# szbonaldo/FedMLP

Measured on AMD Instinct MI355X. Metric: images/sec/client (ICH 224x224 bs=128) at 1/2/4/8 GPUs; mAP vs ref, higher is better.
Workload: dtype f32; 1 GPU; FedMLP stage1 step, Resnet18, ICH-shaped synthetic 3x224x224, C=5, bs=128, one client per GPU, FedAvg all-reduce every 40 steps + once at end; parallelism=clients1, rccl_ranks=1, stream_mode=default: frozen teacher + weight gradients on the engine's side stream, arithmetic=fp32 operands+sums; products as 6 exact bf16 partials on the bf16 matrix pipe

## Files before the change

fedmlp_amd/_lib.py:

```python
import ctypes as C
import os

_HERE = os.path.dirname(os.path.abspath(__file__))
LIB_PATH = os.environ.get("FEDMLP_HIP_LIB") or os.path.join(_HERE, "libfedmlp_hip.so")

FM_MAX_CLASSES = 32
FM_MAX_GROUPS = 8
FM_COMM_ID_BYTES = 128


class FmConfig(C.Structure):
    _fields_ = [("model", C.c_int32), ("n_classes", C.c_int32), ("in_h", C.c_int32),
                ("in_w", C.c_int32), ("max_images", C.c_int32), ("reserved", C.c_int32 * 3),
                ("stream", C.c_void_p)]


class FmAdam(C.Structure):
    _fields_ = [("lr", C.c_float), ("beta1", C.c_float), ("beta2", C.c_float),
                ("eps", C.c_float), ("weight_decay", C.c_float)]


class FmSgd(C.Structure):
    _fields_ = [("lr", C.c_float), ("momentum", C.c_float), ("dampening", C.c_float),
                ("weight_decay", C.c_float), ("nesterov", C.c_int32)]
# ... 98 lines not shown
    "fm_debug_conv_fwd": (C.c_int, [_P, _I32, _P, _P, _I32, _I32, _P, _P, _P, _I32, _P, _P, _P, _P]),
    "fm_debug_block_dgrad": (C.c_int, [_P, _I32, _P, _P, _P, _I32]),
    "fm_debug_conv_planes": (C.c_int, [_P, _I32, _P, _I32, _P, _P, _P, _P, _I32, _P, _P]),
    "fm_debug_conv_arm": (C.c_int, [_P, _I32, _I32, _I32]),
    "fm_debug_pw": (C.c_int, [_P, _I32, _I32, _P, _P, _P, _I32, _I32, _P, _P, _P, _P]),
    "fm_debug_pw_fwd": (C.c_int, [_P, _I32, _P, _P, _I32, _I32, _P, _P, _P, _I32, _P, _P, _P, _P]),
    "fm_debug_proj_bwd": (C.c_int, [_P, _I32, _I32, _P, _P, _P, _P, _P, _I32, _I32, _P, _P]),
    "fm_debug_exp_bwd": (C.c_int, [_P, _I32, _P, _P, _P, _P, _P, _I32, _I32, _P, _P]),
    "fm_debug_get_grads": (C.c_int, [_P, _P]),
    "fm_debug_optim_arena": (C.c_int, [_P, _I32, C.POINTER(_P), C.POINTER(_I64)]),
    "fm_debug_entry_spans": (C.c_int, [_P, _P, _I32]),
    "fm_debug_activation": (C.c_int, [_P, _I32, _I32, _I32, _P, C.POINTER(_I32)]),
    "fm_debug_stem_masks": (C.c_int, [_P, _I32, _I32, _P, _P]),
    "fm_debug_lose_part": (C.c_int, [_I32]),
    "fm_debug_ew": (C.c_int, [_P, _I32, C.POINTER(_P), C.POINTER(_I32), _F]),
    "fm_debug_eff": (C.c_int, [_P, _I32, C.POINTER(_P), C.POINTER(_I32), _F]),
    "fm_debug_eff_ws": (C.c_int, [_I32, C.POINTER(_I32), C.POINTER(C.c_int64)]),
    "fm_debug_head": (C.c_int, [_P, _I32, C.POINTER(_P), C.POINTER(_I32), _F]),
}

_lib = None


def load():
    global _lib
    if _lib is not None:
        return _lib
    if not os.path.exists(LIB_PATH):
        raise RuntimeError(
            f"{LIB_PATH} is missing: the HIP extension is not built and fedmlp_amd has no CPU "
# ... 32 lines not shown
```

fedmlp_amd/csrc/engine.hip:

```cpp
#include <math.h>
#include <stdio.h>
#include <string.h>

#include <algorithm>
#include <string>
#include <unordered_map>
#include <vector>

#include "../../include/fedmlp_hip.h"
#include "../../include/fedmlp_hip_debug.h"
#include "comm.h"
#include "common.h"
#include "kernels.h"
#include "pwconv.h"

static thread_local std::string g_err;
const char* fm_last_error(void) { return g_err.c_str(); }
const char* fm_version(void) { return "fedmlp_hip 0.2 (gfx950)"; }

#define HIPCHK(x)                                                                              \
    do {                                                                                       \
        hipError_t e_ = (x);                                                                   \
        if (e_ != hipSuccess) {                                                                \
            char b_[512];                                                                      \
// ... 157 lines not shown
    size_t NP = 0, NS = 0;
    size_t off_fcw = 0, off_fcb = 0, off_gamma = 0, off_beta = 0, off_rm = 0, off_rv = 0;
    int64_t nf_sd = 0, ni_sd = 0;
    float *grad = nullptr, *adam_m = nullptr, *adam_v = nullptr;
    float* stage_sd = nullptr;
    fm_adam hp{3e-5f, 0.9f, 0.999f, 1e-8f, 5e-4f};
    int64_t adam_t = 0;
    float *x4 = nullptr, *dyh0 = nullptr;
    float* x3 = nullptr;
    bool stem_rows = false;
    unsigned short* x3p = nullptr;
    long long x3p_plane_elems = 0;
    uint8_t* idx0 = nullptr;
    float *GA = nullptr, *GB = nullptr, *GC = nullptr, *GD = nullptr, *GE = nullptr;
    float *ws_stats = nullptr, *ws_part = nullptr;
    int stats_conv = -1, stats_tiles_n = 0;
    size_t slab_floats = 0;
    float *ca = nullptr, *cb = nullptr, *cc = nullptr;
    float *feat = nullptr, *logits = nullptr, *tfeat = nullptr, *tlogits = nullptr, *dlogits = nullptr;
    float* psum = nullptr;
    int64_t *pcnt = nullptr, *tcnt = nullptr;
    float* zeros = nullptr;
    int *sel_counts = nullptr, *sel_top = nullptr, *sel_bot = nullptr, *cls_dev = nullptr;
    int sel_cap = 0;
    int* tag_buf = nullptr;
    size_t tag_buf_ints = 0;
    bool prof = false, prof_fail = false;
    hipError_t soft_err = hipSuccess;
    int* dev_err = nullptr;
    int* host_err = nullptr;
    int* host_err_dev = nullptr;
    bool oprof = false;
    int ctx = -1;
// ... 656 lines not shown
        DALLOC(e->GA, pooled); DALLOC(e->GB, pooled); DALLOC(e->GC, pooled); DALLOC(e->GD, pooled); DALLOC(e->GE, pooled);
    } else {
        const EffSizes z = eff_sizes(e);
        AALLOC(e->GA, z.g_io); AALLOC(e->GB, z.g_io);
        AALLOC(e->T_small, z.t_small); AALLOC(e->T_big, z.t_big);
        DALLOC(e->se_dgp, B * z.max_ce); DALLOC(e->se_drp, B * z.max_cs); DALLOC(e->se_ds, B * z.max_ce);
        side = side && side_fits(e);
        DALLOC(e->hfeat, B * e->D);
    }
    DALLOC(e->ws_stats, max_stats);
    DALLOC(e->ws_part, (size_t)2 * (1024 + 32) * 2 * e->maxC);
    e->slab_floats = std::max<size_t>(max_slab * 8, (size_t)48 << 20);
    DALLOC(e->main.ws_slab, e->slab_floats);
    e->main.rec = e->main.ws_slab;
    DALLOC(e->ca, 2 * e->maxC); DALLOC(e->cb, 2 * e->maxC); DALLOC(e->cc, 2 * e->maxC);
    DALLOC(e->feat, B * e->D); DALLOC(e->tfeat, B * e->D);
    DALLOC(e->logits, B * e->C); DALLOC(e->tlogits, B * e->C); DALLOC(e->dlogits, B * e->C);
    DALLOC(e->psum, (size_t)2 * e->C * e->D); DALLOC(e->pcnt, 2 * e->C); DALLOC(e->tcnt, e->C);
    DALLOC(e->sel_counts, 2); DALLOC(e->cls_dev, FM_MAX_CLASSES);
    DALLOC(e->zeros, 64);
    if (e->planes) {
        const size_t pooled = B * (c0.hout / 2) * (c0.wout / 2) * 64;
        PALLOC(e->GBp, pooled); PALLOC(e->GCp, pooled); PALLOC(e->GDp, pooled);
        size_t mx = 0;
        for (auto& c : e->convs) {
            if (c.cin == 3) continue;
            mx = std::max(mx, std::max(B * c.hin * c.win * c.cin_p, B * c.hout * c.wout * c.cout_p));
        }
        e->xp_scratch_elems = mx * 3;
        float* t3 = nullptr;
// ... 440 lines not shown
            int imgs_per_group, bool frozen, bool z_is_relu_of_bn = false, unsigned short* dyp = nullptr, const unsigned short* zh = nullptr)
{
    const Conv& c = e->convs[bi];
    Bn& b = e->bns[bi];
    const int pix = imgs_per_group * c.hout * c.wout;
    const char* fy = getenv("FM_BN_MASK_FROM_Y");
    const int from_y = fy ? atoi(fy) : 1;
    const float *msc = nullptr, *msh = nullptr;
    if (z_is_relu_of_bn && (z || zh) && (from_y || !z)) { msc = b.scale; msh = b.shift; z = nullptr; zh = nullptr; }
    k_bn_bwd_reduce(dz, z, c.y, b.mean, b.istd, e->ws_part, groups, pix, b.C, L.st, msc, msh, zh);
    k_bn_bwd_finalize(e->ws_part, groups, bn_bwd_blocks(pix), b.C, pix, e->student.state + e->off_gamma + b.ch_off, b.mean,
                      b.istd, e->ca, e->cb, e->cc, e->grad + e->off_gamma + b.ch_off,
                      e->grad + e->off_beta + b.ch_off, L.st, frozen);
    if (dyp) k_bn_bwd_apply_planes(dz, z, c.y, e->ca, e->cb, e->cc, dy, dyp, dyh_out, groups, pix, b.C, L.st, msc, msh, zh);
    else k_bn_bwd_apply(dz, z, c.y, e->ca, e->cb, e->cc, dy, dyh_out, groups, pix, b.C, L.st, msc, msh);
}

void to_nhwc4(fm_engine* e, Lane& L, const float* const* xs, int groups, int B)
{
    if (e->precision && e->model == 1) {
        const Conv& c = e->convs[e->c_stem];
        for (int g = 0; g < groups; ++g)
            k_stem_im2col(xs[g], reinterpret_cast<bf16*>(e->stem_col) + (size_t)g * B * c.hout * c.wout * c.Kw, B, e->H, e->W, c.hout,
                          c.wout, c.k, c.stride, c.pad, c.pad, L.st);
        return;
    }
    if (e->convs[0].stem3) {
        const Conv& c = e->convs[0];
        for (int g = 0; g < groups; ++g)
            k_frame_nhwc3(xs[g], e->x3 + (size_t)g * B * c.Hp * c.Wp * 3, B, e->H, e->W, c.Hp, c.Wp, 3, 3, 0, L.st,
// ... 386 lines not shown
    if (first > nb + 1) return;
    e->ctx = 500;
    { OP(L, "k_fc_bwd"); k_fc_bwd(e->dlogits, e->feat, S + e->off_fcw, nullptr, e->grad + e->off_fcw, e->grad + e->off_fcb, e->GA, DT_F32, imgs,
             512, e->C, cl.hout * cl.wout, L.st, bw.dfeat); }
    float *ga = e->GA, *ge = e->GE;
    for (int b = nb - 1; b >= 0 && 1 + b >= first; --b) {
        const Block& blk = e->blocks[b];
        e->ctx = 400 + b;
        const BlockActs& a = A.blk[b];
        const int par = b & 1;
        float *GB = GBp[par], *GC = GCp[par], *GD = GDp[par];
        unsigned short *gbp = pm ? PB[par] : nullptr, *gcp = pm ? PC[par] : nullptr, *gdp = pm ? PD[par] : nullptr;
        const float* in = b == 0 ? A.p0 : A.blk[b - 1].out;
        const bool last = b + 1 == (int)e->blocks.size();
        side_guard(e, 0, par);
        { OP(L, "bn_bwd");
          if (pm && !last) bn_bwd(e, L, blk.c2, ga, nullptr, nullptr, ga, groups, B, bw.frozen, false, gbp, a.outp);
          else bn_bwd(e, L, blk.c2, ga, a.out, pm ? nullptr : GB, ga, groups, B, bw.frozen, false, gbp); }
        if (blk.ds >= 0) { side_guard(e, 1, par); OP(L, "bn_bwd"); bn_bwd(e, L, blk.ds, ga, nullptr, pm ? nullptr : GC, nullptr, groups, B, bw.frozen, false, gcp); }
        side_guard(e, 2, par);
        { OP(L, "conv_dgrad"); conv_dgrad(e, L, blk.c2, GB, GD, imgs, nullptr, false, gbp); }
        if (conv_on(e, tr, blk.c2)) {
            Lane& SL = side(0, par);
            { OP(SL, "conv_wgrad"); conv_wgrad(e, SL, blk.c2, a.z1, GB, imgs, nullptr, 0, pm ? a.z1p : nullptr, gbp); }
            side_end(e, 0, par);
        }
        { OP(L, "bn_bwd");
          if (pm) bn_bwd(e, L, blk.c1, GD, nullptr, nullptr, nullptr, groups, B, bw.frozen, true, gdp, a.z1p);
          else bn_bwd(e, L, blk.c1, GD, a.z1, GD, nullptr, groups, B, bw.frozen, true); }
        { OP(L, "conv_dgrad");
          if (blk.ds >= 0) {
              if (!block_dgrad(e, L, blk.c1, blk.ds, GD, GC, ge, imgs, gdp, gcp)) {
                  conv_dgrad(e, L, blk.ds, GC, ge, imgs, nullptr, false, gcp);
                  conv_dgrad(e, L, blk.c1, GD, ge, imgs, nullptr, true, gdp);
// ... 2195 lines not shown
        k_bn_bwd_finalize(F(0), d[0], d[1], d[2], d[3], F(1), F(2), F(3), F(4), F(5), F(6), F(7), F(8), s, d[4] != 0);
        break;
    case FM_EW_BN_BWD_APPLY:
    case FM_EW_BN_BWD_APPLY_PLANES: {
        const bool pl = op == FM_EW_BN_BWD_APPLY_PLANES;
        ARGCHK(need({0, 2, 3, 4, 5}) && pos(3) && d[2] % 4 == 0 && (!p[8] == !p[9]), "bn_bwd_apply: C % 4, mask_scale with mask_shift");
        if (pl) {
            ARGCHK(d[2] % 32 == 0 && p[10], "bn_bwd_apply_planes: C % 32, dyp");
            k_bn_bwd_apply_planes(F(0), F(1), F(2), F(3), F(4), F(5), F(6), U(10), F(7), d[0], d[1], d[2], s, F(8), F(9), U(11));
        } else {
            ARGCHK(p[6], "bn_bwd_apply: dy");
            k_bn_bwd_apply(F(0), F(1), F(2), F(3), F(4), F(5), F(6), F(7), d[0], d[1], d[2], s, F(8), F(9));
        }
        break;
    }
    default:
        ARGCHK(false, "op");
    }
    HIPCHK(hipGetLastError());
    HIPCHK(hipStreamSynchronize(s));
    return FM_OK;
}

static const char* eff_dims_bad(int32_t op, const int32_t* d)
{
    auto pos = [&](int a, int b) { for (int i = a; i < b; ++i) if (d[i] < 1) return false; return true; };
    if (op == FM_EFF_DW_FWD || op == FM_EFF_DW_DGRAD || op == FM_EFF_DW_WGRAD) {
        if (d[0] != DT_F32 && d[0] != DT_BF16) return "dt";
        if (!pos(1, 7) || d[12] < 1) return "a dimension < 1";
        if (d[6] % 4) return "C % 4";
        if (d[7] != 3 && d[7] != 5) return "K is 3 or 5";
        if (d[8] != 1 && d[8] != 2) return "stride is 1 or 2";
        if (d[4] != (d[2] + d[8] - 1) / d[8] || d[5] != (d[3] + d[8] - 1) / d[8]) return "Ho, Wo = ceil(Hi, Wi / stride)";
        if (d[9] < 0 || d[9] >= d[7] || d[10] < 0 || d[10] >= d[7]) return "pad_t, pad_l in 0 .. K-1";
        if (d[11] < 0 || d[11] > 2) return "act";
// ... 214 lines not shown
```

fedmlp_amd/csrc/kernels.h:

```cpp
#pragma once
#include <hip/hip_runtime.h>
#include <stdint.h>

#include "common.h"

#define FM_MAXC 32

struct ClassVec { float v[FM_MAXC]; };
struct TapList { int t[9]; int n; };

void k_nchw_to_nhwc4(const float* x, float* y, int imgs, int H, int W, hipStream_t s);
void k_stem_im2col(const float* x, void* col, int imgs, int H, int W, int Ho, int Wo, int k, int stride, int pad_t, int pad_l,
                   hipStream_t s);
void k_oihw_to_ohwi(const float* src, float* dst, int O, int I, int H, int W, int Wpad, int Ipad, hipStream_t s, int Ostride = 0);
void k_ohwi_to_oihw(const float* src, float* dst, int O, int I, int H, int W, int Wpad, int Ipad, hipStream_t s, int Ostride = 0);
void k_stem3_mask_grad(float* g, int O, hipStream_t s);
void k_frame_nhwc3(const float* x, float* y, int imgs, int H, int W, int Hp, int Wp, int top, int left, int src_nhwc3,
                   hipStream_t s, unsigned short* yp = nullptr, long long yp_plane_elems = 0);
void k_pack_dgrad(const float* w, float* out, int Co, int T, int Ci, TapList taps, hipStream_t s);
struct PackJob { long long w_off; float* out; int Co, T, Ci, ntaps; int taps[9]; int blk0; };
void k_pack_dgrad_all(const float* state, const PackJob* jobs, int njobs, int nblocks, hipStream_t s);
int pack_job_blocks(int Co, int Ci, int ntaps);
struct SplitJob { long long src_off; const float* src; long long dst_off; int M, nkb, blk0; };
void k_split_weights(const float* src_base, unsigned short* dst_base, const SplitJob* jobs, int njobs, int nblocks, hipStream_t s);
int split_job_blocks(int M, int nkb);
struct SplitJobBM { long long src_off; const float* src; long long dst_off; int M, ntaps, cib, blk0; };
void k_split_weights_bm(const float* src_base, unsigned short* dst_base, const SplitJobBM* jobs, int njobs, int nblocks, hipStream_t s);
int split_job_bm_blocks(int M, int nsteps);
void k_split_planes(const float* x, unsigned short* dst, long long npix, int C, hipStream_t s);
void k_planes_to_f32(const unsigned short* src, float* x, long long npix, int C, hipStream_t s);
void k_bn_apply_planes(const float* y, const float* scale, const float* shift, const float* res, const float* y2, const float* scale2,
                       const float* shift2, float* out, unsigned short* outp, int groups, int pix_per_group, int C, int relu,
                       hipStream_t s, const unsigned short* resp = nullptr);
void k_stem_pool_planes(const float* y, const float* scale, const float* shift, float* pooled, uint8_t* idx, unsigned short* pooledp,
                        int groups, int imgs_per_group, int H, int W, int C, hipStream_t s);
void k_bn_bwd_apply_planes(const float* dz, const float* z, const float* y, const float* ca, const float* cb, const float* cc, float* dy,
                           unsigned short* dyp, float* dyh_out, int groups, int pix_per_group, int C, hipStream_t s,
                           const float* mask_scale = nullptr, const float* mask_shift = nullptr, const unsigned short* zh = nullptr);
void k_scale(float* x, float w, int64_t n, hipStream_t s);
#define FM_FOLD_MAX 16
struct FoldArgs { const float* s[FM_FOLD_MAX]; float n[FM_FOLD_MAX]; };
void k_fedavg_fold(const FoldArgs& a, int K, float tot, float* out, int64_t n, hipStream_t s);
void k_axpby(float* y, const float* x, float a, float b, int64_t n, hipStream_t s);
#define FM_DIST_CHUNK 8192
struct DistEntry { long long off; int len, row, dense, Ipad, I, Wpad, W, chunk0, nchunks, all_real; };
struct DistChunk { int entry, start; };
void k_state_dist(const FoldArgs& a, int K, const float* ref, const DistEntry* ent, int n_entries, const DistChunk* chunks,
                  int n_chunks, int64_t NS, double* part, float* norms, hipStream_t s);

#define FM_METRICS_ROWS 64
#define FM_METRICS_BP 256
#define FM_METRICS_TILE 2048
size_t fm_metrics_ws_bytes(int64_t N, int C);
// ... 171 lines not shown
```

fedmlp_amd/csrc/planes_ew.hip:

```cpp
#include "common.h"
#include "kernels.h"
#include "split3.h"

static inline int pe_cdiv(int64_t a, int64_t b) { return (int)((a + b - 1) / b); }

#if __HIP_DEVICE_COMPILE__
__device__ __forceinline__ size_t pe_off(int c, int64_t pix, int64_t P)
{
    return (((size_t)(c >> 5) * 3) * P + pix) * 64 + ((c & 15) >> 2) * 16 + ((c >> 4) & 1) * 8;
}
__device__ __forceinline__ void pe_store_planes(unsigned short* planes, int64_t P, int c, int64_t pix, f32x4 v, bool active)
{
    f32x4 up;
#pragma unroll
    for (int k = 0; k < 4; ++k) up[k] = __shfl_down(v[k], 4);
    if (active && (c & 16) == 0) {
        sp_u32x4 H, M, L;
        split3(v, up, H, M, L);
        unsigned char* d = reinterpret_cast<unsigned char*>(planes) + (((size_t)(c >> 5) * 3) * P + pix) * 64 + ((c & 15) >> 2) * 16;
        *reinterpret_cast<sp_u32x4*>(d) = H;
        *reinterpret_cast<sp_u32x4*>(d + (size_t)P * 64) = M;
        *reinterpret_cast<sp_u32x4*>(d + (size_t)P * 128) = L;
    }
}
// ... 163 lines not shown
    if (active) {
        if (dyh_out) st4(dyh_out + o, d);
        if (dy) st4(dy + o, r);
    }
    pe_store_planes(dyp, P, c, pix, r, active);
#endif
}
void k_bn_bwd_apply_planes(const float* dz, const float* z, const float* y, const float* ca, const float* cb, const float* cc, float* dy,
                           unsigned short* dyp, float* dyh_out, int groups, int pix_per_group, int C, hipStream_t s,
                           const float* mask_scale, const float* mask_shift, const unsigned short* zh)
{
    const int64_t n4 = (int64_t)pix_per_group * (C / 4);
    hipLaunchKernelGGL(bn_bwd_apply_planes_kernel, dim3(pe_cdiv(n4, 256), groups), dim3(256), 0, s, dz, z, y, ca, cb, cc, dy, dyp,
                       dyh_out, pix_per_group, C, mask_scale, mask_shift, zh);
}
```

fedmlp_amd/csrc/pwgrad.hip:

```cpp
#include <stdlib.h>

#include <algorithm>
#include <type_traits>

#include "common.h"
#include "kernels.h"
#include "split3.h"

#if __HIP_DEVICE_COMPILE__
template <int IMM> __device__ __forceinline__ uint2 pw_read_tr(unsigned addr)
{
    uint2 v;
    asm volatile("ds_read_b64_tr_b16 %0, %1 offset:%2" : "=v"(v) : "v"(addr), "n"(IMM));
    return v;
}
#endif

template <int N, typename F> __device__ __forceinline__ void pw_for(F f)
{
    f(std::integral_constant<int, 0>{});
    if constexpr (N > 1) f(std::integral_constant<int, 1>{});
    if constexpr (N > 2) f(std::integral_constant<int, 2>{});
    if constexpr (N > 3) f(std::integral_constant<int, 3>{});
}
template <int FR, int FC, int SP>
__global__ __launch_bounds__(512, 2) void pwgrad_kernel(const PwgradParams p)
{
#if __HIP_DEVICE_COMPILE__
    constexpr int WN = 4;
    constexpr int BM = 32 * FR, BN = 64 * FC;
    constexpr int NBA = BM / 32, NBB = BN / 32;
    constexpr int SA = NBA * 6144, SB = NBB * 6144;
    constexpr int JA = (NBA * 3 + 3) / 4, JB = (NBB * 3 + 3) / 4;
    typedef __attribute__((address_space(3))) void lds_void;
    extern __shared__ __attribute__((aligned(16))) unsigned char smem[];
    const int tid = threadIdx.x;
    const int lane = tid & 63, wave = __builtin_amdgcn_readfirstlane(tid >> 6);
    const int wm = wave / WN, wn = wave % WN;
    const int li = lane & 15, lg = lane >> 4;
    const unsigned lds0 = (unsigned)(size_t)smem;
    const unsigned As = lds0, Bs = lds0 + 2 * SA;

    const int tile = blockIdx.x, split = blockIdx.y;
    const int tm = tile % p.tilesM, tn = tile / p.tilesM;
    const int m0 = tm * BM;
    const int jb0 = tn * NBB;
    const int cib = p.Ci >> 5;
    const long long pbeg = (long long)split * p.pix_per_split;
    const long long pend = min(p.npix, pbeg + p.pix_per_split);
    const int nsteps = (int)((pend - pbeg + 31) >> 5);
    const int Wi = p.Wi, Hi = p.Hi, Wo = p.Wo, Ho = p.Ho;

    constexpr unsigned OOB = 0x80000000u;
    const int h16 = wave & 1, q4 = wave >> 1;
    const int drow = 16 * h16 + (lane >> 2);
    const int chunk = (lane & 3) ^ (((drow >> 3) & 1) << 1);
    const __amdgpu_buffer_rsrc_t rsA = __builtin_amdgcn_make_buffer_rsrc(
        const_cast<unsigned short*>(p.dYp), 0, (unsigned)((size_t)(p.M >> 5) * 3 * p.npix * 64), 0x00020000);
    const int shift = p.pad * (Wi + 1);
    const __amdgpu_buffer_rsrc_t rsB = __builtin_amdgcn_make_buffer_rsrc(
        const_cast<unsigned char*>(reinterpret_cast<const unsigned char*>(p.Xp) - (size_t)shift * 64), 0,
        (unsigned)(((size_t)cib * 3 * p.xpix + shift) * 64), 0x00020000);
    const unsigned voffA0 = (unsigned)(drow * 64 + chunk * 16);
    int r_img, r_oh, r_ow;
// ... 170 lines not shown

#pragma unroll
    for (int r = 0; r < FR; ++r) {
        const int tM = wm * FR + r;
        const int jm = 16 * (tM & 1) + li, gm = jm >> 3, wi = jm & 7;
        const int m = m0 + 32 * (tM >> 1) + (wi < 4 ? 4 * gm + wi : 16 + 4 * gm + (wi - 4));
        if (m >= p.M) continue;
#pragma unroll
        for (int c = 0; c < FC; ++c) {
            const int tN = wn * FC + c;
            const int jb = jb0 + (tN >> 1);
            if (jb >= p.nblk_n) continue;
            const int gn = 2 * (tN & 1) + (lg >> 1);
            const int n = jb * 32 + ((lg & 1) ? 16 + 4 * gn : 4 * gn);
            *reinterpret_cast<f32x4*>(p.slab + ((size_t)split * p.M + m) * p.Nw + n) = acc[r][c];
        }
    }
#endif
}

int pwgrad_tile_m(int M) { return M >= 128 ? 128 : 64; }
int pwgrad_tile_nb(int nblk_n) { return (nblk_n % 8 != 0 && nblk_n % 6 == 0) ? 6 : 8; }
bool pwgrad_takes(int M, int Ci, int ksz, long long npix, long long xpix, int Wi, int pad)
{
    if (M % 64 != 0 || (M > 64 && M % 128 != 0) || Ci % 32 != 0 || !((ksz == 3 && pad == 1) || (ksz == 1 && pad == 0))) return false;
    return ((long long)(Ci >> 5) * 3 * xpix + 2 * (Wi + 1)) * 64 < 0x7ff00000LL && (long long)(M >> 5) * 3 * npix * 64 < 0x7ff00000LL;
}

int launch_pwgrad(PwgradParams p, size_t slab_floats, hipStream_t s)
{
    static bool attr_done = false;
    constexpr int L44 = 2 * (4 + 8) * 6144, L43 = 2 * (4 + 6) * 6144, L24 = 2 * (2 + 8) * 6144, L23 = 2 * (2 + 6) * 6144;
    if (!attr_done) {
#define PW_ATTR(FR_, FC_, SP_, L_) set_max_dyn_lds(reinterpret_cast<const void*>(&pwgrad_kernel<FR_, FC_, SP_>), L_, "pwgrad_kernel")
        PW_ATTR(4, 4, 6, L44); PW_ATTR(4, 3, 6, L43); PW_ATTR(2, 4, 6, L24); PW_ATTR(2, 3, 6, L23);
        PW_ATTR(4, 4, 9, L44); PW_ATTR(4, 3, 9, L43); PW_ATTR(2, 4, 9, L24); PW_ATTR(2, 3, 9, L23);
#undef PW_ATTR
        attr_done = true;
    }
    p.nblk_n = p.ksz * p.ksz * (p.Ci >> 5);
    const int nb = pwgrad_tile_nb(p.nblk_n), bm = pwgrad_tile_m(p.M);
    p.tilesM = p.M / bm;
    p.tilesN = (p.nblk_n + nb - 1) / nb;
    const int tiles = p.tilesM * p.tilesN;
    int splits = std::max(1, 256 / tiles);
    splits = (int)std::min<long long>(splits, std::max<long long>(1, p.npix / 256));
    splits = (int)std::min<size_t>(splits, std::max<size_t>(1, slab_floats / ((size_t)p.M * p.Nw)));
    p.pix_per_split = (int)((((p.npix + splits - 1) / splits) + 31) & ~31LL);
    splits = (int)((p.npix + p.pix_per_split - 1) / p.pix_per_split);
    dim3 grid(tiles, splits);
#define PW_LAUNCH(FR_, FC_, L_)                                                                              \
    do {                                                                                                     \
        if (p.sp == 9) hipLaunchKernelGGL((pwgrad_kernel<FR_, FC_, 9>), grid, dim3(512), L_, s, p);          \
        else hipLaunchKernelGGL((pwgrad_kernel<FR_, FC_, 6>), grid, dim3(512), L_, s, p);                    \
    } while (0)
    if (bm == 128) { if (nb == 8) PW_LAUNCH(4, 4, L44); else PW_LAUNCH(4, 3, L43); }
    else           { if (nb == 8) PW_LAUNCH(2, 4, L24); else PW_LAUNCH(2, 3, L23); }
#undef PW_LAUNCH
    return splits;
}
// ... 1 lines not shown
```

fedmlp_amd/engine.py:

```python
import ctypes as C

import numpy as np
import torch

from . import _lib, spec

MODEL_IDS = {"Resnet18": 0, "Efficient_b0": 1}
PRECISION_IDS = {"fp32": 0, "bf16": 1}
PRODUCT_FORMS = {None: 0, 6: 3, 0: 1, 9: 2}


def _ptr(t):
    if t is None:
        return None
    assert t.is_cuda and t.is_contiguous() and t.dtype in (torch.float32, torch.int32, torch.bfloat16), \
        (t.device, t.dtype, t.is_contiguous())
    return C.c_void_p(t.data_ptr())


class Engine:

    def __init__(self, model, n_classes, in_h, in_w, max_images, device=None, precision="fp32", streams=0, products=None):
        if not torch.cuda.is_available():
            raise RuntimeError("fedmlp_amd.Engine needs a GPU (no CPU fallback)")
# ... 759 lines not shown
    CONV_ARMS = ("igemm", "igemm_stem", "stem_rows", "pconv_ts", "pconv_tap", "pwgrad", "pwgrad_ring", "wgrad_generic",
                 "wgrad_skinny", "stem_dgrad")

    def debug_conv_arm(self, op, conv, imgs):
        rc = self.lib.fm_debug_conv_arm(self.h, op, conv, imgs)
        if rc < 0:
            _lib.check(rc)
        return self.CONV_ARMS[rc]

    def debug_block_dgrad(self, block, dy1, dyd, dx, imgs):
        self._enqueue()
        _lib.check(self.lib.fm_debug_block_dgrad(self.h, block, _ptr(dy1), _ptr(dyd), _ptr(dx), imgs))

    EW_OPS = ("split_planes", "planes_to_f32", "bn_finalize", "bn_finalize_frozen", "bn_eval_affine", "bn_apply",
              "bn_apply_planes", "stem_pool", "stem_pool_planes", "stem_pool_bwd", "stem_pool_bn_reduce", "stem_pool_bn_apply",
              "bn_bwd_reduce", "bn_bwd_finalize", "bn_bwd_apply", "bn_bwd_apply_planes")

    def debug_ew(self, op, ptrs, dims, scalars=()):
        assert len(ptrs) <= 12 and len(dims) <= 5 and len(scalars) <= 2, (len(ptrs), len(dims), len(scalars))
        for t in ptrs:
            assert t is None or (t.is_cuda and t.is_contiguous()), op
        p = (C.c_void_p * 12)(*[None if t is None else t.data_ptr() for t in ptrs])
        d = (C.c_int32 * 5)(*[int(v) for v in dims])
        _lib.check(self.lib.fm_debug_ew(self.h, self.EW_OPS.index(op), p, d, _lib.fvec(list(scalars) + [0.0] * (2 - len(scalars)))))

    EFF_OPS = ("dw_fwd", "dw_dgrad", "dw_wgrad", "se_fwd", "se_scale", "se_bwd_bn1", "se_wgrad", "bnact_apply", "chan_reduce",
               "bnact_bwd_apply")

    def debug_eff_ws(self, op, dims):
        assert len(dims) <= 13, len(dims)
        d = (C.c_int32 * 13)(*[int(v) for v in dims])
# ... 77 lines not shown
```

include/fedmlp_hip_debug.h:

```cpp
#ifndef FEDMLP_HIP_DEBUG_H
#define FEDMLP_HIP_DEBUG_H

#include "fedmlp_hip.h"

#ifdef __cplusplus
extern "C" {
#endif

int fm_debug_conv_info(fm_engine* e, int32_t conv, int32_t* info16);
int fm_debug_num_convs(fm_engine* e);
int fm_debug_conv(fm_engine* e, int32_t op, int32_t conv, const float* x_dev, const float* dy_dev,
                  float* out_dev, int32_t imgs, int32_t groups, float* stats_dev);

int fm_debug_conv_fwd(fm_engine* e, int32_t conv, const float* x_dev, float* out_dev, int32_t imgs, int32_t groups,
                      const float* scale_dev, const float* shift_dev, const float* res_dev, int32_t act, const float* psc_dev,
                      const float* psh_dev, const float* gate_dev, float* stats_dev);

int fm_debug_conv_planes(fm_engine* e, int32_t conv, const uint16_t* xp_dev, int32_t imgs, const float* scale_dev,
                         const float* shift_dev, const float* res_dev, const uint16_t* resp_dev, int32_t relu, float* out_dev,
                         uint16_t* outp_dev);

enum { FM_ARM_IGEMM = 0, FM_ARM_IGEMM_STEM, FM_ARM_STEM_ROWS, FM_ARM_PCONV_TS, FM_ARM_PCONV_TAP, FM_ARM_PWGRAD, FM_ARM_PWGRAD_RING,
       FM_ARM_WGRAD_GENERIC, FM_ARM_WGRAD_SKINNY, FM_ARM_STEM_DGRAD };
int fm_debug_conv_arm(fm_engine* e, int32_t op, int32_t conv, int32_t imgs);
// ... 17 lines not shown

int fm_debug_activation(fm_engine* e, int32_t kind, int32_t block, int32_t imgs, float* host_nhwc,
                        int32_t* dims4);

int fm_debug_stem_masks(fm_engine* e, int32_t imgs, int32_t groups, uint8_t* relu_bits_host, uint8_t* argmax_host);

int fm_debug_lose_part(int32_t on);

int fm_debug_get_grads(fm_engine* e, float* host_f32);
int fm_debug_optim_arena(fm_engine* e, int32_t which, float** dev_ptr, int64_t* numel);
int fm_debug_entry_spans(fm_engine* e, int64_t* off_len, int32_t n_entries);

enum {
    FM_EW_SPLIT_PLANES = 0, FM_EW_PLANES_TO_F32, FM_EW_BN_FINALIZE, FM_EW_BN_FINALIZE_FROZEN, FM_EW_BN_EVAL_AFFINE, FM_EW_BN_APPLY,
    FM_EW_BN_APPLY_PLANES, FM_EW_STEM_POOL, FM_EW_STEM_POOL_PLANES, FM_EW_STEM_POOL_BWD, FM_EW_STEM_POOL_BN_REDUCE,
    FM_EW_STEM_POOL_BN_APPLY, FM_EW_BN_BWD_REDUCE, FM_EW_BN_BWD_FINALIZE, FM_EW_BN_BWD_APPLY, FM_EW_BN_BWD_APPLY_PLANES
};
#define FM_EW_NPTR 12
#define FM_EW_NDIM 5
#define FM_EW_NSCAL 2
int fm_debug_ew(fm_engine* e, int32_t op, void* const* p, const int32_t* d, const float* sc);

enum { FM_EFF_DW_FWD = 0, FM_EFF_DW_DGRAD, FM_EFF_DW_WGRAD, FM_EFF_SE_FWD, FM_EFF_SE_SCALE, FM_EFF_SE_BWD_BN1, FM_EFF_SE_WGRAD,
       FM_EFF_BNACT_APPLY, FM_EFF_CHAN_REDUCE, FM_EFF_BNACT_BWD_APPLY };
#define FM_EFF_NPTR 16
#define FM_EFF_NDIM 13
#define FM_EFF_NWS 4
int fm_debug_eff(fm_engine* e, int32_t op, void* const* p, const int32_t* d, const float* sc);
int fm_debug_eff_ws(int32_t op, const int32_t* d, int64_t* floats);

enum { FM_HD_AVGPOOL = 0, FM_HD_FC_FWD, FM_HD_FC_BWD, FM_HD_LOSS_BCE, FM_HD_LOSS_STAGE1, FM_HD_LOSS_STAGE2, FM_HD_LOSS_FIXMATCH };
#define FM_HD_NPTR 8
#define FM_HD_NDIM 5
#define FM_HD_NSCAL 2
int fm_debug_head(fm_engine* e, int32_t op, void* const* p, const int32_t* d, const float* sc);

// ... 5 lines not shown
```

Measured before the change: 6175 images/sec.

## Fuse paired BN backward for main and downsample branches; balance pwgrad split tail

In downsample blocks, the main-path and shortcut batch-norm backward passes share the same upstream gradient and relu mask. They now run as one paired reduce kernel and one paired apply kernel, so dz and the mask are read once instead of twice and two launches are saved. Separately, the pointwise weight-gradient kernel gains a range mode for the 128x8 tile shape. It spreads leftover pixel steps across idle blocks to even out the load, and zeroes any unused slab partitions. This adds index arithmetic, extra slab partitions and more complex code in exchange for better occupancy on underfilled grids.

```diff
diff --git a/fedmlp_amd/_lib.py b/fedmlp_amd/_lib.py
--- a/fedmlp_amd/_lib.py
+++ b/fedmlp_amd/_lib.py
@@ -136,6 +136,7 @@
     "fm_debug_stem_masks": (C.c_int, [_P, _I32, _I32, _P, _P]),
     "fm_debug_lose_part": (C.c_int, [_I32]),
     "fm_debug_ew": (C.c_int, [_P, _I32, C.POINTER(_P), C.POINTER(_I32), _F]),
+    "fm_debug_bn_pair": (C.c_int, [_P, _I32]),
     "fm_debug_eff": (C.c_int, [_P, _I32, C.POINTER(_P), C.POINTER(_I32), _F]),
     "fm_debug_eff_ws": (C.c_int, [_I32, C.POINTER(_I32), C.POINTER(C.c_int64)]),
     "fm_debug_head": (C.c_int, [_P, _I32, C.POINTER(_P), C.POINTER(_I32), _F]),
diff --git a/fedmlp_amd/csrc/engine.hip b/fedmlp_amd/csrc/engine.hip
--- a/fedmlp_amd/csrc/engine.hip
+++ b/fedmlp_amd/csrc/engine.hip
@@ -195,9 +195,12 @@
     uint8_t* idx0 = nullptr;
     float *GA = nullptr, *GB = nullptr, *GC = nullptr, *GD = nullptr, *GE = nullptr;
     float *ws_stats = nullptr, *ws_part = nullptr;
+    float* ws_part2 = nullptr;
+    bool bn_pair = true;
     int stats_conv = -1, stats_tiles_n = 0;
     size_t slab_floats = 0;
     float *ca = nullptr, *cb = nullptr, *cc = nullptr;
+    float *ca2 = nullptr, *cb2 = nullptr, *cc2 = nullptr;
     float *feat = nullptr, *logits = nullptr, *tfeat = nullptr, *tlogits = nullptr, *dlogits = nullptr;
     float* psum = nullptr;
     int64_t *pcnt = nullptr, *tcnt = nullptr;
@@ -884,6 +887,10 @@
     DALLOC(e->main.ws_slab, e->slab_floats);
     e->main.rec = e->main.ws_slab;
     DALLOC(e->ca, 2 * e->maxC); DALLOC(e->cb, 2 * e->maxC); DALLOC(e->cc, 2 * e->maxC);
+    if (e->model == 0 && e->planes) {
+        DALLOC(e->ws_part2, (size_t)2 * (1024 + 32) * 2 * e->maxC);
+        DALLOC(e->ca2, 2 * e->maxC); DALLOC(e->cb2, 2 * e->maxC); DALLOC(e->cc2, 2 * e->maxC);
+    }
     DALLOC(e->feat, B * e->D); DALLOC(e->tfeat, B * e->D);
     DALLOC(e->logits, B * e->C); DALLOC(e->tlogits, B * e->C); DALLOC(e->dlogits, B * e->C);
     DALLOC(e->psum, (size_t)2 * e->C * e->D); DALLOC(e->pcnt, 2 * e->C); DALLOC(e->tcnt, e->C);
@@ -1354,6 +1361,20 @@
                       e->grad + e->off_beta + b.ch_off, L.st, frozen);
     if (dyp) k_bn_bwd_apply_planes(dz, z, c.y, e->ca, e->cb, e->cc, dy, dyp, dyh_out, groups, pix, b.C, L.st, msc, msh, zh);
     else k_bn_bwd_apply(dz, z, c.y, e->ca, e->cb, e->cc, dy, dyh_out, groups, pix, b.C, L.st, msc, msh);
+}
+
+void bn_bwd_pair(fm_engine* e, Lane& L, int a, int b, const float* dz, const unsigned short* zh, int groups, int imgs_per_group,
+                 bool frozen, unsigned short* dyp_a, unsigned short* dyp_b)
+{
+    const Conv &c1 = e->convs[a], &c2 = e->convs[b];
+    Bn &b1 = e->bns[a], &b2 = e->bns[b];
+    const int pix = imgs_per_group * c1.hout * c1.wout;
+    k_bn_bwd_reduce_pair(dz, zh, c1.y, c2.y, b1.mean, b1.istd, b2.mean, b2.istd, e->ws_part, e->ws_part2, groups, pix, b1.C, L.st);
+    k_bn_bwd_finalize(e->ws_part, groups, bn_bwd_blocks(pix), b1.C, pix, e->student.state + e->off_gamma + b1.ch_off, b1.mean,
+                      b1.istd, e->ca, e->cb, e->cc, e->grad + e->off_gamma + b1.ch_off, e->grad + e->off_beta + b1.ch_off, L.st, frozen);
+    k_bn_bwd_finalize(e->ws_part2, groups, bn_bwd_blocks(pix), b2.C, pix, e->student.state + e->off_gamma + b2.ch_off, b2.mean,
+                      b2.istd, e->ca2, e->cb2, e->cc2, e->grad + e->off_gamma + b2.ch_off, e->grad + e->off_beta + b2.ch_off, L.st, frozen);
+    k_bn_bwd_apply_planes_pair(dz, zh, c1.y, c2.y, e->ca, e->cb, e->cc, e->ca2, e->cb2, e->cc2, dyp_a, dyp_b, groups, pix, b1.C, L.st);
 }
 
 void to_nhwc4(fm_engine* e, Lane& L, const float* const* xs, int groups, int B)
@@ -1770,10 +1791,16 @@
         const float* in = b == 0 ? A.p0 : A.blk[b - 1].out;
         const bool last = b + 1 == (int)e->blocks.size();
         side_guard(e, 0, par);
-        { OP(L, "bn_bwd");
-          if (pm && !last) bn_bwd(e, L, blk.c2, ga, nullptr, nullptr, ga, groups, B, bw.frozen, false, gbp, a.outp);
-          else bn_bwd(e, L, blk.c2, ga, a.out, pm ? nullptr : GB, ga, groups, B, bw.frozen, false, gbp); }
-        if (blk.ds >= 0) { side_guard(e, 1, par); OP(L, "bn_bwd"); bn_bwd(e, L, blk.ds, ga, nullptr, pm ? nullptr : GC, nullptr, groups, B, bw.frozen, false, gcp); }
+        if (pm && !last && blk.ds >= 0 && e->bn_pair) {
+            side_guard(e, 1, par);
+            OP(L, "bn_bwd");
+            bn_bwd_pair(e, L, blk.c2, blk.ds, ga, a.outp, groups, B, bw.frozen, gbp, gcp);
+        } else {
+            { OP(L, "bn_bwd");
+              if (pm && !last) bn_bwd(e, L, blk.c2, ga, nullptr, nullptr, ga, groups, B, bw.frozen, false, gbp, a.outp);
+              else bn_bwd(e, L, blk.c2, ga, a.out, pm ? nullptr : GB, ga, groups, B, bw.frozen, false, gbp); }
+            if (blk.ds >= 0) { side_guard(e, 1, par); OP(L, "bn_bwd"); bn_bwd(e, L, blk.ds, ga, nullptr, pm ? nullptr : GC, nullptr, groups, B, bw.frozen, false, gcp); }
+        }
         side_guard(e, 2, par);
         { OP(L, "conv_dgrad"); conv_dgrad(e, L, blk.c2, GB, GD, imgs, nullptr, false, gbp); }
         if (conv_on(e, tr, blk.c2)) {
@@ -3999,11 +4026,27 @@
         }
         break;
     }
+    case FM_EW_BN_BWD_REDUCE_PAIR:
+        ARGCHK(need({0, 1, 2, 3, 4, 5, 6, 7, 8, 9}) && pos(3) && d[2] % 32 == 0 && d[2] <= 1024 && 1024 % d[2] == 0,
+               "bn_bwd_reduce_pair: C a power of two in 32 .. 1024");
+        k_bn_bwd_reduce_pair(F(0), U(1), F(2), F(3), F(4), F(5), F(6), F(7), F(8), F(9), d[0], d[1], d[2], s);
+        break;
+    case FM_EW_BN_BWD_APPLY_PLANES_PAIR:
+        ARGCHK(need({0, 1, 2, 3, 4, 5, 6, 7, 8, 9, 10, 11}) && pos(3) && d[2] % 32 == 0, "bn_bwd_apply_planes_pair: C % 32");
+        k_bn_bwd_apply_planes_pair(F(0), U(1), F(2), F(3), F(4), F(5), F(6), F(7), F(8), F(9), U(10), U(11), d[0], d[1], d[2], s);
+        break;
     default:
         ARGCHK(false, "op");
     }
     HIPCHK(hipGetLastError());
     HIPCHK(hipStreamSynchronize(s));
+    return FM_OK;
+}
+
+int fm_debug_bn_pair(fm_engine* e, int32_t on)
+{
+    ARGCHK(e, "null engine");
+    e->bn_pair = on != 0;
     return FM_OK;
 }
 
diff --git a/fedmlp_amd/csrc/kernels.h b/fedmlp_amd/csrc/kernels.h
--- a/fedmlp_amd/csrc/kernels.h
+++ b/fedmlp_amd/csrc/kernels.h
@@ -37,6 +37,12 @@
 void k_bn_bwd_apply_planes(const float* dz, const float* z, const float* y, const float* ca, const float* cb, const float* cc, float* dy,
                            unsigned short* dyp, float* dyh_out, int groups, int pix_per_group, int C, hipStream_t s,
                            const float* mask_scale = nullptr, const float* mask_shift = nullptr, const unsigned short* zh = nullptr);
+void k_bn_bwd_reduce_pair(const float* dz, const unsigned short* zh, const float* ya, const float* yb, const float* mean_a,
+                          const float* istd_a, const float* mean_b, const float* istd_b, float* part_a, float* part_b, int groups,
+                          int pix_per_group, int C, hipStream_t s);
+void k_bn_bwd_apply_planes_pair(const float* dz, const unsigned short* zh, const float* ya, const float* yb, const float* ca_a,
+                                const float* cb_a, const float* cc_a, const float* ca_b, const float* cb_b, const float* cc_b,
+                                unsigned short* dyp_a, unsigned short* dyp_b, int groups, int pix_per_group, int C, hipStream_t s);
 void k_scale(float* x, float w, int64_t n, hipStream_t s);
 #define FM_FOLD_MAX 16
 struct FoldArgs { const float* s[FM_FOLD_MAX]; float n[FM_FOLD_MAX]; };
diff --git a/fedmlp_amd/csrc/planes_ew.hip b/fedmlp_amd/csrc/planes_ew.hip
--- a/fedmlp_amd/csrc/planes_ew.hip
+++ b/fedmlp_amd/csrc/planes_ew.hip
@@ -201,3 +201,127 @@
     hipLaunchKernelGGL(bn_bwd_apply_planes_kernel, dim3(pe_cdiv(n4, 256), groups), dim3(256), 0, s, dz, z, y, ca, cb, cc, dy, dyp,
                        dyh_out, pix_per_group, C, mask_scale, mask_shift, zh);
 }
+
+__global__ __launch_bounds__(256) void bn_bwd_reduce_pair_kernel(const float* __restrict__ dz, const unsigned short* __restrict__ zh,
+                                                                 const float* __restrict__ ya, const float* __restrict__ yb,
+                                                                 const float* __restrict__ mean_a, const float* __restrict__ istd_a,
+                                                                 const float* __restrict__ mean_b, const float* __restrict__ istd_b,
+                                                                 float* __restrict__ part_a, float* __restrict__ part_b,
+                                                                 int pix_per_group, int C, long long zP)
+{
+#if __HIP_DEVICE_COMPILE__
+    __shared__ f32x4 red[2][256];
+    const int g = blockIdx.y, nblk = gridDim.x;
+    const int Q = C >> 2, P = 256 / Q;
+    const int cq = threadIdx.x % Q, pl = threadIdx.x / Q;
+    const int TP = 8 * P;
+    const size_t base = (size_t)g * pix_per_group * C;
+    const f32x4 mu = *reinterpret_cast<const f32x4*>(mean_a + g * C + cq * 4);
+    const f32x4 is = *reinterpret_cast<const f32x4*>(istd_a + g * C + cq * 4);
+    const f32x4 mub = *reinterpret_cast<const f32x4*>(mean_b + g * C + cq * 4);
+    const f32x4 isb = *reinterpret_cast<const f32x4*>(istd_b + g * C + cq * 4);
+    f32x4 s1 = {0.f, 0.f, 0.f, 0.f}, s2 = {0.f, 0.f, 0.f, 0.f}, s3 = {0.f, 0.f, 0.f, 0.f};
+    for (int t0 = blockIdx.x * TP; t0 < pix_per_group; t0 += nblk * TP)
+#pragma unroll 2
+    for (int p = t0 + pl; p < min(pix_per_group, t0 + TP); p += P) {
+        const size_t o = base + (size_t)p * C + cq * 4;
+        f32x4 d = *reinterpret_cast<const f32x4*>(dz + o);
+        const int c = cq * 4;
+        const uint2 hb = *reinterpret_cast<const uint2*>(reinterpret_cast<const unsigned char*>(zh) +
+            ((size_t)(c >> 5) * 3 * zP + (size_t)g * pix_per_group + p) * 64 + ((c & 15) >> 2) * 16 + ((c >> 4) & 1) * 8);
+        d[0] = (short)(hb.x & 0xffffu) > 0 ? d[0] : 0.f;
+        d[1] = (short)(hb.x >> 16) > 0 ? d[1] : 0.f;
+        d[2] = (short)(hb.y & 0xffffu) > 0 ? d[2] : 0.f;
+        d[3] = (short)(hb.y >> 16) > 0 ? d[3] : 0.f;
+        const f32x4 yy = *reinterpret_cast<const f32x4*>(ya + o);
+        const f32x4 xh = (yy - mu) * is;
+        s1 += d;
+        s2 += d * xh;
+        const f32x4 yyb = *reinterpret_cast<const f32x4*>(yb + o);
+        const f32x4 xhb = (yyb - mub) * isb;
+        s3 += d * xhb;
+    }
+    red[0][threadIdx.x] = s1;
+    red[1][threadIdx.x] = s2;
+    __syncthreads();
+    if (pl == 0) {
+        for (int k = 1; k < P; ++k) {
+            s1 += red[0][k * Q + cq];
+            s2 += red[1][k * Q + cq];
+        }
+    }
+    __syncthreads();
+    red[0][threadIdx.x] = s3;
+    __syncthreads();
+    if (pl == 0) {
+        for (int k = 1; k < P; ++k) s3 += red[0][k * Q + cq];
+        float* oa = part_a + ((size_t)(g * nblk + blockIdx.x) * 2) * C + cq * 4;
+        float* ob = part_b + ((size_t)(g * nblk + blockIdx.x) * 2) * C + cq * 4;
+        *reinterpret_cast<f32x4*>(oa) = s1;
+        *reinterpret_cast<f32x4*>(oa + C) = s2;
+        *reinterpret_cast<f32x4*>(ob) = s1;
+        *reinterpret_cast<f32x4*>(ob + C) = s3;
+    }
+#endif
+}
+void k_bn_bwd_reduce_pair(const float* dz, const unsigned short* zh, const float* ya, const float* yb, const float* mean_a,
+                          const float* istd_a, const float* mean_b, const float* istd_b, float* part_a, float* part_b, int groups,
+                          int pix_per_group, int C, hipStream_t s)
+{
+    hipLaunchKernelGGL(bn_bwd_reduce_pair_kernel, dim3(bn_bwd_blocks(pix_per_group), groups), dim3(256), 0, s, dz, zh, ya, yb, mean_a,
+                       istd_a, mean_b, istd_b, part_a, part_b, pix_per_group, C, (long long)groups * pix_per_group);
+}
+
+#if __HIP_DEVICE_COMPILE__
+__device__ __forceinline__ f32x4 pe_bn_bwd_dy(f32x4 a, f32x4 d, f32x4 b, f32x4 yy, f32x4 c)
+{
+    f32x4 r;
+#pragma unroll
+    for (int k = 0; k < 4; ++k) {
+        const float t = b[k] * yy[k];
+        r[k] = __builtin_fmaf(a[k], d[k], t) + c[k];
+    }
+    return r;
+}
+#endif
+__global__ __launch_bounds__(256) void bn_bwd_apply_planes_pair_kernel(const float* __restrict__ dz, const unsigned short* __restrict__ zh,
+                                                                       const float* __restrict__ ya, const float* __restrict__ yb,
+                                                                       const float* __restrict__ ca, const float* __restrict__ cb_,
+                                                                       const float* __restrict__ cc, const float* __restrict__ ca2,
+                                                                       const float* __restrict__ cb2, const float* __restrict__ cc2,
+                                                                       unsigned short* __restrict__ dyp_a, unsigned short* __restrict__ dyp_b,
+                                                                       int pix_per_group, int C)
+{
+#if __HIP_DEVICE_COMPILE__
+    const int grp = blockIdx.y;
+    const int Q = C >> 2;
+    const int64_t n4 = (int64_t)pix_per_group * Q;
+    const int64_t P = (int64_t)gridDim.y * pix_per_group;
+    const int64_t i = (int64_t)blockIdx.x * 256 + threadIdx.x;
+    const bool active = i < n4;
+    const int64_t ii = active ? i : 0;
+    const int c = (int)(ii % Q) * 4;
+    const int64_t pix = (int64_t)grp * pix_per_group + ii / Q;
+    const size_t o = (size_t)pix * C + c;
+    f32x4 d = ld4(dz + o);
+    d = pe_mask_h(d, zh, P, c, pix);
+    {
+        const f32x4 yy = ld4(ya + o);
+        const f32x4 r = pe_bn_bwd_dy(ld4(ca + grp * C + c), d, ld4(cb_ + grp * C + c), yy, ld4(cc + grp * C + c));
+        pe_store_planes(dyp_a, P, c, pix, r, active);
+    }
+    {
+        const f32x4 yy = ld4(yb + o);
+        const f32x4 r = pe_bn_bwd_dy(ld4(ca2 + grp * C + c), d, ld4(cb2 + grp * C + c), yy, ld4(cc2 + grp * C + c));
+        pe_store_planes(dyp_b, P, c, pix, r, active);
+    }
+#endif
+}
+void k_bn_bwd_apply_planes_pair(const float* dz, const unsigned short* zh, const float* ya, const float* yb, const float* ca_a,
+                                const float* cb_a, const float* cc_a, const float* ca_b, const float* cb_b, const float* cc_b,
+                                unsigned short* dyp_a, unsigned short* dyp_b, int groups, int pix_per_group, int C, hipStream_t s)
+{
+    const int64_t n4 = (int64_t)pix_per_group * (C / 4);
+    hipLaunchKernelGGL(bn_bwd_apply_planes_pair_kernel, dim3(pe_cdiv(n4, 256), groups), dim3(256), 0, s, dz, zh, ya, yb, ca_a, cb_a,
+                       cc_a, ca_b, cb_b, cc_b, dyp_a, dyp_b, pix_per_group, C);
+}
diff --git a/fedmlp_amd/csrc/pwgrad.hip b/fedmlp_amd/csrc/pwgrad.hip
--- a/fedmlp_amd/csrc/pwgrad.hip
+++ b/fedmlp_amd/csrc/pwgrad.hip
@@ -23,7 +23,7 @@
     if constexpr (N > 2) f(std::integral_constant<int, 2>{});
     if constexpr (N > 3) f(std::integral_constant<int, 3>{});
 }
-template <int FR, int FC, int SP>
+template <int FR, int FC, int SP, bool RANGE = false>
 __global__ __launch_bounds__(512, 2) void pwgrad_kernel(const PwgradParams p)
 {
 #if __HIP_DEVICE_COMPILE__
@@ -41,13 +41,41 @@
     const unsigned lds0 = (unsigned)(size_t)smem;
     const unsigned As = lds0, Bs = lds0 + 2 * SA;
 
-    const int tile = blockIdx.x, split = blockIdx.y;
+    const int S = (int)((p.npix + 31) >> 5);
+    const int tiles = p.tilesM * p.tilesN;
+    const int ms = (int)gridDim.x / tiles, nmain = ms * tiles, nleft = (int)gridDim.x - nmain;
+    const int m0 = (int)((long long)tiles * S / gridDim.x), m = m0 + m0 / 36, R = S - ms * m;
+    const int lb = (int)blockIdx.x - nmain;
+    const long long Lt = (long long)tiles * R;
+    const long long g0 = RANGE && lb >= 0 ? lb * Lt / nleft : 0, g1 = RANGE && lb >= 0 ? (lb + 1) * Lt / nleft : 0;
+    const int nseg = RANGE && lb >= 0 ? (int)((g1 - 1) / R - g0 / R) + 1 : 1;
+  for (int seg = 0; seg < nseg; ++seg) {
+    int tile = blockIdx.x, split = blockIdx.y;
+    long long pbeg = (long long)split * p.pix_per_split;
+    long long pend = min(p.npix, pbeg + p.pix_per_split);
+    bool ends_tile = false;
+    if constexpr (RANGE) {
+        if (lb < 0) {
+            tile = (int)blockIdx.x % tiles;
+            split = (int)blockIdx.x / tiles;
+            pbeg = (long long)split * m * 32;
+            pend = pbeg + (long long)m * 32;
+        } else {
+            tile = (int)(g0 / R) + seg;
+            const long long tb = (long long)tile * R;
+            pbeg = ((long long)ms * m + max(g0, tb) - tb) * 32;
+            pend = min(p.npix, ((long long)ms * m + min(g1, tb + R) - tb) * 32);
+            ends_tile = g1 >= tb + R;
+            long long bf = tb * nleft / Lt;
+            if ((bf + 1) * Lt / nleft <= tb) ++bf;
+            split = ms + (int)(lb - bf);
+            if (seg) __builtin_amdgcn_s_barrier();
+        }
+    }
     const int tm = tile % p.tilesM, tn = tile / p.tilesM;
     const int m0 = tm * BM;
     const int jb0 = tn * NBB;
     const int cib = p.Ci >> 5;
-    const long long pbeg = (long long)split * p.pix_per_split;
-    const long long pend = min(p.npix, pbeg + p.pix_per_split);
     const int nsteps = (int)((pend - pbeg + 31) >> 5);
     const int Wi = p.Wi, Hi = p.Hi, Wo = p.Wo, Ho = p.Ho;
 
@@ -248,8 +276,14 @@
             const int gn = 2 * (tN & 1) + (lg >> 1);
             const int n = jb * 32 + ((lg & 1) ? 16 + 4 * gn : 4 * gn);
             *reinterpret_cast<f32x4*>(p.slab + ((size_t)split * p.M + m) * p.Nw + n) = acc[r][c];
-        }
-    }
+            if constexpr (RANGE) {
+                if (ends_tile)
+                    for (int z = split + 1; z < p.splits; ++z)
+                        *reinterpret_cast<f32x4*>(p.slab + ((size_t)z * p.M + m) * p.Nw + n) = f32x4{0.f, 0.f, 0.f, 0.f};
+            }
+        }
+    }
+  }
 #endif
 }
 
@@ -270,6 +304,8 @@
         PW_ATTR(4, 4, 6, L44); PW_ATTR(4, 3, 6, L43); PW_ATTR(2, 4, 6, L24); PW_ATTR(2, 3, 6, L23);
         PW_ATTR(4, 4, 9, L44); PW_ATTR(4, 3, 9, L43); PW_ATTR(2, 4, 9, L24); PW_ATTR(2, 3, 9, L23);
 #undef PW_ATTR
+        set_max_dyn_lds(reinterpret_cast<const void*>(&pwgrad_kernel<4, 4, 6, true>), L44, "pwgrad_kernel");
+        set_max_dyn_lds(reinterpret_cast<const void*>(&pwgrad_kernel<4, 4, 9, true>), L44, "pwgrad_kernel");
         attr_done = true;
     }
     p.nblk_n = p.ksz * p.ksz * (p.Ci >> 5);
@@ -278,6 +314,30 @@
     p.tilesN = (p.nblk_n + nb - 1) / nb;
     const int tiles = p.tilesM * p.tilesN;
     int splits = std::max(1, 256 / tiles);
+    if (bm == 128 && nb == 8 && tiles * splits * 10 < 256 * 9) {
+        const int nblocks = 256;
+        const int S = (int)((p.npix + 31) >> 5);
+        const int m0 = (int)((long long)tiles * S / nblocks), m = m0 + m0 / 36, R = S - splits * m;
+        const int nleft = nblocks - tiles * splits;
+        const long long Lt = (long long)tiles * R;
+        auto block_of = [&](long long step) {
+            long long b = step * nleft / Lt;
+            if ((b + 1) * Lt / nleft <= step) ++b;
+            return b;
+        };
+        int nslabs = 0;
+        if (m >= 8 && R >= 1 && Lt >= nleft) {
+            for (int t = 0; t < tiles; ++t)
+                nslabs = std::max(nslabs, splits + (int)(block_of((long long)(t + 1) * R - 1) - block_of((long long)t * R)) + 1);
+        }
+        if (nslabs > 0 && (size_t)nslabs * p.M * p.Nw <= slab_floats) {
+            p.splits = nslabs;
+            p.pix_per_split = 0;
+            if (p.sp == 9) hipLaunchKernelGGL((pwgrad_kernel<4, 4, 9, true>), dim3(nblocks), dim3(512), L44, s, p);
+            else hipLaunchKernelGGL((pwgrad_kernel<4, 4, 6, true>), dim3(nblocks), dim3(512), L44, s, p);
+            return nslabs;
+        }
+    }
     splits = (int)std::min<long long>(splits, std::max<long long>(1, p.npix / 256));
     splits = (int)std::min<size_t>(splits, std::max<size_t>(1, slab_floats / ((size_t)p.M * p.Nw)));
     p.pix_per_split = (int)((((p.npix + splits - 1) / splits) + 31) & ~31LL);
diff --git a/fedmlp_amd/engine.py b/fedmlp_amd/engine.py
--- a/fedmlp_amd/engine.py
+++ b/fedmlp_amd/engine.py
@@ -797,7 +797,11 @@
 
     EW_OPS = ("split_planes", "planes_to_f32", "bn_finalize", "bn_finalize_frozen", "bn_eval_affine", "bn_apply",
               "bn_apply_planes", "stem_pool", "stem_pool_planes", "stem_pool_bwd", "stem_pool_bn_reduce", "stem_pool_bn_apply",
-              "bn_bwd_reduce", "bn_bwd_finalize", "bn_bwd_apply", "bn_bwd_apply_planes")
+              "bn_bwd_reduce", "bn_bwd_finalize", "bn_bwd_apply", "bn_bwd_apply_planes", "bn_bwd_reduce_pair",
+              "bn_bwd_apply_planes_pair")
+
+    def debug_bn_pair(self, on):
+        _lib.check(self.lib.fm_debug_bn_pair(self.h, int(bool(on))))
 
     def debug_ew(self, op, ptrs, dims, scalars=()):
         assert len(ptrs) <= 12 and len(dims) <= 5 and len(scalars) <= 2, (len(ptrs), len(dims), len(scalars))
diff --git a/include/fedmlp_hip_debug.h b/include/fedmlp_hip_debug.h
--- a/include/fedmlp_hip_debug.h
+++ b/include/fedmlp_hip_debug.h
@@ -55,12 +55,15 @@
 enum {
     FM_EW_SPLIT_PLANES = 0, FM_EW_PLANES_TO_F32, FM_EW_BN_FINALIZE, FM_EW_BN_FINALIZE_FROZEN, FM_EW_BN_EVAL_AFFINE, FM_EW_BN_APPLY,
     FM_EW_BN_APPLY_PLANES, FM_EW_STEM_POOL, FM_EW_STEM_POOL_PLANES, FM_EW_STEM_POOL_BWD, FM_EW_STEM_POOL_BN_REDUCE,
-    FM_EW_STEM_POOL_BN_APPLY, FM_EW_BN_BWD_REDUCE, FM_EW_BN_BWD_FINALIZE, FM_EW_BN_BWD_APPLY, FM_EW_BN_BWD_APPLY_PLANES
+    FM_EW_STEM_POOL_BN_APPLY, FM_EW_BN_BWD_REDUCE, FM_EW_BN_BWD_FINALIZE, FM_EW_BN_BWD_APPLY, FM_EW_BN_BWD_APPLY_PLANES,
+    FM_EW_BN_BWD_REDUCE_PAIR, FM_EW_BN_BWD_APPLY_PLANES_PAIR
 };
 #define FM_EW_NPTR 12
 #define FM_EW_NDIM 5
 #define FM_EW_NSCAL 2
 int fm_debug_ew(fm_engine* e, int32_t op, void* const* p, const int32_t* d, const float* sc);
+
+int fm_debug_bn_pair(fm_engine* e, int32_t on);
 
 enum { FM_EFF_DW_FWD = 0, FM_EFF_DW_DGRAD, FM_EFF_DW_WGRAD, FM_EFF_SE_FWD, FM_EFF_SE_SCALE, FM_EFF_SE_BWD_BN1, FM_EFF_SE_WGRAD,
        FM_EFF_BNACT_APPLY, FM_EFF_CHAN_REDUCE, FM_EFF_BNACT_BWD_APPLY };
```

Measured after the change: 6191 images/sec (median of 2 runs). Within noise of the previous version (+0.3%).
